# takahiroharada/OCLRadixSort

Hardware: AMD Instinct MI355X
Metric: Gkeys/s on uniform-random u32 keys; achieved % of HBM-read roofline (higher is better)
Workload: dtype u32; 1 GPU; Key-only RadixSort32, 67108864 uniform-random u32 keys (splitmix64 hi32, seed 123+step), 1xMI355X, in place; keys_per_gpu=67108864, parallelism=1 GPU, sort_algo=auto, digit_bits=8

## Files before the change

### oclradixsort_amd/csrc/hybrid_kernels.hpp

```cpp
#pragma once
#include <hip/hip_runtime.h>
#include <stdint.h>

#include "radix_kernels.hpp"
#include "onesweep_kernels.hpp"
#include "dict_kernels.hpp"
#include "dict_big_kernels.hpp"

namespace adlhip {

__device__ __forceinline__ bool grid_barrier(uint32_t* counter, uint32_t& target, uint32_t wgs, uint32_t* fault, bool data_fence = true)
{
    __shared__ uint32_t ok;
    if (!data_fence) asm volatile("s_waitcnt vmcnt(0)" ::: "memory");
    __syncthreads();
    if (threadIdx.x == 0) {
        if (data_fence) __builtin_amdgcn_fence(__ATOMIC_RELEASE, "agent");
        asm volatile("s_waitcnt vmcnt(0)" ::: "memory");
        __hip_atomic_fetch_add(counter, 1u, __ATOMIC_RELAXED, __HIP_MEMORY_SCOPE_AGENT);
        target += wgs;
        uint32_t spins = 0u, good = 1u;
        while (__hip_atomic_load(counter, __ATOMIC_RELAXED, __HIP_MEMORY_SCOPE_AGENT) < target) {
            if (++spins > (1u << 24)) { good = 0u; break; }
            __builtin_amdgcn_s_sleep(2);
// ... 977 lines not shown
        E* __restrict__ dst = out + seg_off[sg(seg)];
        auto prefetch_next = [&]() {
            if (more) {
                const S* __restrict__ src = in + (size_t)next * in_stride;
#pragma unroll
                for (int j = 0; j < K; ++j)
                    if ((uint32_t)(j * NT + tid) < m_next && m_next <= (uint32_t)CAP) e[j] = load_once(src + j * NT + tid);
            }
        };
        const bool sortable = m != 0u && m <= (uint32_t)CAP && low_bits != 0u;
        if (m > (uint32_t)CAP && tid == 0) atomicOr(fault + 1, 0x40000u);
#pragma unroll
        for (int i = 0; i < WPT; ++i) s_cnt[tid + i * NT] = 0u;
        lds_barrier();
        uint32_t rk2[(K + 1) / 2];
#pragma unroll
        for (int j = 0; j < (K + 1) / 2; ++j) rk2[j] = 0u;
        bool hard = false;
        if (sortable) {
#pragma unroll
            for (int j = 0; j < K; ++j) {
                if ((uint32_t)(j * NT + tid) < m) {
                    const uint32_t b = bin_of(e[j]);
                    const uint32_t hs = (b & 1u) << 4;
                    const uint32_t old = __hip_atomic_fetch_add(&s_cnt[b >> 1], 1u << hs, __ATOMIC_RELAXED, __HIP_MEMORY_SCOPE_WORKGROUP);
                    const uint32_t r = (old >> hs) & 0xffffu;
                    rk2[j >> 1] |= r << (16 * (j & 1));
                    hard |= r >= kBinLimit;
                }
            }
        }
        if (lane == 0) s_hard[w] = 0u;
        if (__any(hard) && lane == 0) s_hard[w] = 1u;
        lds_barrier();
        bool is_hard = false;
#pragma unroll
        for (int i = 0; i < NW; ++i) is_hard |= s_hard[i] != 0u;
        if (is_hard && tid == 0) hard_list[__hip_atomic_fetch_add(hard_cnt, 1u, __ATOMIC_RELAXED, __HIP_MEMORY_SCOPE_AGENT)] = seg;
        if (!is_hard && sortable) {
            {
                uint32_t wv[WPT];
                uint32_t sum = 0u;
#pragma unroll
                for (int i = 0; i < WPT; ++i) {
                    wv[i] = s_cnt[tid * WPT + i];
                    sum += (wv[i] & 0xffffu) + (wv[i] >> 16);
                }
                const uint32_t inc = wave_incl_scan_u32(sum);
                if (lane == 63) s_wsum[w] = inc;
                lds_barrier();
                uint32_t run = inc - sum;
#pragma unroll
                for (int i = 0; i < NW; ++i)
                    if (i < w) run += s_wsum[i];
#pragma unroll
                for (int i = 0; i < WPT; ++i) {
                    const uint32_t c0 = wv[i] & 0xffffu, c1 = wv[i] >> 16;
                    const uint32_t lo = run;
                    run += c0;
                    const uint32_t hi = run;
                    run += c1;
                    s_cnt[tid * WPT + i] = lo | (hi << 16);
                }
            }
            lds_barrier();
#pragma unroll
            for (int j = 0; j < K; ++j)
                if ((uint32_t)(j * NT + tid) < m) s_buf[(uint32_t)s_start[bin_of(e[j])] + ((rk2[j >> 1] >> (16 * (j & 1))) & 0xffffu)] = e[j];
            prefetch_next();
            lds_barrier();
#pragma unroll
            for (int j = 0; j < K; ++j) {
                const uint32_t p = (uint32_t)(j * NT + tid);
                if (p < m) {
                    const S x = s_buf[p];
                    const uint32_t b = bin_of(x);
                    const uint32_t lo = s_start[b];
                    const uint32_t hi = b == dmask ? m : (uint32_t)s_start[b + 1u];
                    uint32_t f = p;
                    if (hi - lo > 1u) {
                        uint32_t c = 0u;
                        for (uint32_t q = lo; q < hi; ++q) {
                            const S y = s_buf[q];
                            c += (y < x || (y == x && q < p)) ? 1u : 0u;
                        }
                        f = lo + c;
                    }
                    dst[f] = (E)x | hi_bits;
                }
            }
            lds_barrier();
        } else {
            if (!is_hard && m != 0u && m <= (uint32_t)CAP) {
#pragma unroll
                for (int j = 0; j < K; ++j) {
                    const uint32_t p = (uint32_t)(j * NT + tid);
                    if (p < m) dst[p] = (E)e[j] | hi_bits;
                }
            }
            prefetch_next();
        }
        if (!more) break;
        seg = next;
        m = m_next;
    }
}

struct StablePlace {
    uint32_t top;
    uint32_t low_bits;
    uint32_t sort_bits;
    uint32_t pad;
    unsigned long long prefix;
    unsigned long long kmask;
};

template <bool KEY64, typename E>
__device__ __forceinline__ unsigned long long key_of(E e)
{
    if constexpr (KEY64) return (unsigned long long)e;
    else return (unsigned long long)(uint32_t)e;
}

template <typename E>
struct BucketPass {
    const E* src;
    E* dst;
    uint32_t* cursors;
    uint32_t cursor_shift;
    uint32_t src_count_shift;
    uint32_t* flag;
    const uint32_t* src_counts;
    uint32_t n;
    uint32_t src_stride;
    uint32_t tiles_per_bucket;
    uint32_t dst_stride;
    uint32_t dst_total;
    int start_bit;
    uint32_t* zero_me;
    const uint32_t* sample;
    int which_digit;
    int dst16;
    const StablePlace* place;
    const uint32_t* status_a;
    uint32_t pieces, rows_per_chain_a, slice;
    uint32_t seg_shift;
    uint32_t* tickets;
};

struct Msd2Placement {
    int top;
    unsigned long long prefix;
};
__device__ __forceinline__ Msd2Placement msd2_placement(const uint32_t* __restrict__ sample )
{
    const unsigned long long o = ((unsigned long long)sample[1] << 32) | sample[0];
    const unsigned long long a = ((unsigned long long)sample[3] << 32) | sample[2];
    const unsigned long long diff = o ^ a;
    Msd2Placement p;
    p.top = diff ? 64 - __builtin_clzll(diff) : 0;
    if (p.top < 16) p.top = 16;
    p.prefix = p.top < 64 ? (o >> p.top) : 0ull;
    return p;
}
__device__ __forceinline__ size_t probe_sample_index(uint32_t k, uint32_t n)
{
    const uint32_t cell = n >> 14;
    const uint32_t hash24 = (uint32_t)(((unsigned long long)k * 0x9E3779B97F4A7C15ull) >> 40);
    const uint32_t jit = (uint32_t)(((unsigned long long)hash24 * cell) >> 24);
    unsigned long long at = (unsigned long long)k * (unsigned long long)n / 16384ull + jit;
    if (at >= n) at = n - 1u;
    return (size_t)at;
}
ADLHIP_KERNEL __global__ __launch_bounds__(1024) void probe_positions_selftest_kernel(uint32_t n, uint32_t* __restrict__ out)
{
    uint32_t hi = 0u, bad = 0u;
    for (int i = 0; i < 16; ++i) {
        const uint32_t k = threadIdx.x * 16u + (uint32_t)i;
        const unsigned long long at = probe_sample_index(k, n);
        const unsigned long long lo = (unsigned long long)k * n / 16384ull, up = (unsigned long long)(k + 1u) * n / 16384ull;
        if (at < lo || at >= (up > lo ? up : lo + 1ull) || at >= n) ++bad;
        hi = at > hi ? (uint32_t)at : hi;
    }
    atomicMax(out + 0, hi);
    if (bad) atomicAdd(out + 1, bad);
}

constexpr int kSampleWGs = 16;
constexpr int kSamples = 2048;
constexpr int kSampleArriveWord = 13;

__device__ __forceinline__ size_t sample_position(int k, uint32_t n)
{
    const unsigned long long lo = (unsigned long long)k * n / (unsigned)kSamples, hi = (unsigned long long)(k + 1) * n / (unsigned)kSamples;
    uint32_t h = (uint32_t)k * 0x85EBCA6Bu + 0x27D4EB2Fu;
    h ^= h >> 15;
    h *= 0xC2B2AE35u;
    h ^= h >> 13;
    return (size_t)(lo + (((unsigned long long)h * (hi - lo)) >> 32));
}

__device__ __forceinline__ void sample_accumulate(unsigned long long v0, unsigned long long v1, uint32_t* sample, uint32_t* flag)
{
    const int lane = (int)threadIdx.x;
    unsigned long long o = v0 | v1, a = v0 & v1;
#pragma unroll
    for (int sh = 32; sh >= 1; sh >>= 1) {
        o |= __shfl_xor(o, sh);
        a &= __shfl_xor(a, sh);
    }
    if (lane == 0) {
        __hip_atomic_fetch_or(sample + 0, (uint32_t)o, __ATOMIC_RELAXED, __HIP_MEMORY_SCOPE_AGENT);
        __hip_atomic_fetch_or(sample + 1, (uint32_t)(o >> 32), __ATOMIC_RELAXED, __HIP_MEMORY_SCOPE_AGENT);
        __hip_atomic_fetch_and(sample + 2, (uint32_t)a, __ATOMIC_RELAXED, __HIP_MEMORY_SCOPE_AGENT);
        __hip_atomic_fetch_and(sample + 3, (uint32_t)(a >> 32), __ATOMIC_RELAXED, __HIP_MEMORY_SCOPE_AGENT);
    }
    __shared__ uint32_t s_seen[256];
#pragma unroll
    for (int i = 0; i < 4; ++i) s_seen[i * 64 + lane] = 0u;
    uint32_t mine = 0u;
#pragma unroll
    for (int j = 0; j < 2; ++j) {
        const unsigned long long hv = ((j ? v1 : v0) + 0x632BE59BD9B4E019ull) * 0x9E3779B97F4A7C15ull;
        const uint32_t fp = (uint32_t)(hv >> 32) | 1u;
        uint32_t h = (uint32_t)(hv >> 24) & 255u;
        for (int step = 0; step < 256; ++step) {
            const uint32_t old = atomicCAS(&s_seen[h], 0u, fp);
            if (old == 0u) break;
            if (old == fp) {
                ++mine;
                break;
            }
            h = (h + 1u) & 255u;
        }
    }
    uint32_t reps = mine;
#pragma unroll
    for (int sh = 32; sh >= 1; sh >>= 1) reps += __shfl_xor(reps, sh);
    if (lane == 0 && reps) __hip_atomic_fetch_add(flag + kSampleRepeatsWord, reps, __ATOMIC_RELAXED, __HIP_MEMORY_SCOPE_AGENT);
}

template <typename E>
__global__ __launch_bounds__(64) void msd2_sample_kernel(const E* __restrict__ src, uint32_t n, uint32_t* sample, uint32_t* bar,
                                                         uint32_t* fault, uint32_t* flag, uint32_t dup_thr)
{
    const int tid = (int)(blockIdx.x * 64u + threadIdx.x);
    if (tid == 0) {
        __hip_atomic_store(bar, 0u, __ATOMIC_RELAXED, __HIP_MEMORY_SCOPE_AGENT);
        fault[0] = 0u;
        __hip_atomic_store(flag + kSampleThresholdWord, dup_thr, __ATOMIC_RELAXED, __HIP_MEMORY_SCOPE_AGENT);
    }
    if (tid < kTileTicketCounters)
        __hip_atomic_store(flag + kTileTicketWord0 + kTileTicketStride * tid, 0u, __ATOMIC_RELAXED, __HIP_MEMORY_SCOPE_AGENT);
    const E x0 = src[sample_position(2 * tid, n)], x1 = src[sample_position(2 * tid + 1, n)];
    sample_accumulate((unsigned long long)x0, (unsigned long long)x1, sample, flag);
}

template <typename E, int NT, int K, int PASS>
__global__ __launch_bounds__(NT) void msd_bucket_scatter_kernel(BucketPass<E> a)
{
    using C = TileCfg<E, 8, NT, K>;
    typedef AosIO<E> IO;
    constexpr int BINS = 256;
    constexpr int NW = C::NW;
    extern __shared__ __attribute__((aligned(16))) unsigned char smem[];
    E* __restrict__ s_elems = reinterpret_cast<E*>(smem + C::OFF_ELEMS);
    uint32_t* __restrict__ s_wcnt = reinterpret_cast<uint32_t*>(smem + C::OFF_WCNT);
    uint32_t* __restrict__ s_goff = reinterpret_cast<uint32_t*>(smem + C::OFF_GOFF);
    if (a.zero_me && blockIdx.x == 0 && threadIdx.x == 0) __hip_atomic_store(a.zero_me, 0u, __ATOMIC_RELAXED, __HIP_MEMORY_SCOPE_AGENT);
    uint32_t give_up = 0u;
    if constexpr (PASS >= 1) {
        if (threadIdx.x == 0) give_up = large_sort_gave_up(a.flag);
    }
    uint32_t base, valid, cursor_base = 0u;
    uint32_t lin = 0u;
    if constexpr (PASS == 3) {
        uint32_t* __restrict__ s_misc = reinterpret_cast<uint32_t*>(smem + C::OFF_MISC);
        const uint32_t b = blockIdx.x / a.tiles_per_bucket, t = blockIdx.x % a.tiles_per_bucket;
        if (threadIdx.x < 64u) {
            const int l = (int)threadIdx.x;
            uint32_t cnt = 0u;
            if ((uint32_t)l < a.pieces) {
                const uint32_t c0 = (uint32_t)l * a.slice;
                if (c0 < a.n) {
                    const uint32_t len = (c0 + a.slice < a.n ? c0 + a.slice : a.n) - c0;
                    const uint32_t rows = (len + (uint32_t)C::TILE - 1u) / (uint32_t)C::TILE;
                    cnt = a.status_a[((size_t)l * a.rows_per_chain_a + rows - 1u) * BINS + b] & kValMask;
                    if (cnt > a.src_stride) cnt = a.src_stride;
                }
            }
            const uint32_t incl = wave_incl_scan_u32(cnt);
            const uint32_t total = (uint32_t)__builtin_amdgcn_readlane((int)incl, 63);
            if (l < 32) {
                const bool real = (uint32_t)l < a.pieces;
                s_goff[l] = real ? incl : 0xffffffffu;
                s_goff[32 + l] = real ? (b * a.pieces + (uint32_t)l) * a.src_stride - (incl - cnt) : 0u;
            }
            const uint32_t pos = t * (uint32_t)C::TILE;
            uint32_t v = 0u;
            if (pos < total) v = total - pos < (uint32_t)C::TILE ? total - pos : (uint32_t)C::TILE;
            const unsigned long long after = __ballot((uint32_t)l < a.pieces && incl > pos && cnt != 0u);
            uint32_t ln = 0xffffffffu, split = 0u, ln2 = 0u;
            if (after && v != 0u) {
                const int c0 = __builtin_ctzll(after);
                const uint32_t end0 = (uint32_t)__builtin_amdgcn_readlane((int)incl, c0);
                const uint32_t first0 = end0 - (uint32_t)__builtin_amdgcn_readlane((int)cnt, c0);
                const unsigned long long rest = after & ~(1ull << c0);
                if (pos + v <= end0) {
                    ln = (b * a.pieces + (uint32_t)c0) * a.src_stride + (pos - first0);
                    split = v;
                } else if (rest) {
                    const int c1 = __builtin_ctzll(rest);
                    const uint32_t end1 = (uint32_t)__builtin_amdgcn_readlane((int)incl, c1);
                    if (pos + v <= end1) {
                        ln = (b * a.pieces + (uint32_t)c0) * a.src_stride + (pos - first0);
                        split = end0 - pos;
// ... 53 lines not shown
        uint32_t c = 0u;
        for (uint32_t i = 0; i < a.pieces; ++i) c += (q0 >= s_end[i]) ? 1u : 0u;
        const int rem = (int)valid - (int)wbase;
#pragma unroll
        for (int j = 0; j < K; ++j) {
            const uint32_t q = q0 + (uint32_t)(j * 64);
            while (c < 31u && q >= s_end[c]) ++c;
            e[j] = (j * 64 < rem) ? load_once(a.src + (size_t)(q + s_adj[c])) : ~E(0);
        }
    } else if (PASS == 3 && reinterpret_cast<const uint32_t*>(smem + C::OFF_MISC)[4] < valid) {
        const uint32_t split = reinterpret_cast<const uint32_t*>(smem + C::OFF_MISC)[4];
        const uint32_t ln2 = reinterpret_cast<const uint32_t*>(smem + C::OFF_MISC)[5];
        const int rem = (int)valid - (int)wbase;
#pragma unroll
        for (int j = 0; j < K; ++j) {
            const uint32_t i = wbase + (uint32_t)(j * 64);
            e[j] = (j * 64 < rem) ? load_once(a.src + (size_t)((i < split ? lin : ln2) + i)) : ~E(0);
        }
    } else {
        const typename IO::Cursor p = io.cursor((size_t)(PASS == 3 ? lin : base) + wbase);
        if (valid == (uint32_t)C::TILE) {
#pragma unroll
            for (int j = 0; j < K; ++j) e[j] = p.at(j * 64);
        } else {
            const int rem = (int)valid - (int)wbase;
#pragma unroll
            for (int j = 0; j < K; ++j) e[j] = (j * 64 < rem) ? p.at(j * 64) : ~E(0);
        }
    }
    if (a.sample && a.which_digit == 1 && place.top < (int)(8 * sizeof(E))) {
        const E pre = (E)place.prefix;
        const int rem = (int)valid - (int)wbase;
        E bad = E(0);
#pragma unroll
        for (int j = 0; j < K; ++j)
            if (j * 64 < rem) bad |= (e[j] >> place.top) ^ pre;
        if (bad != E(0)) __hip_atomic_fetch_or(a.flag, 1u, __ATOMIC_RELAXED, __HIP_MEMORY_SCOPE_AGENT);
    }
#pragma unroll
    for (int b = lane; b < BINS; b += 64) my_wcnt[b] = 0u;
    uint32_t rnk2[(K + 1) / 2];
    {
        uint32_t rnk[K];
        rank_in_wave<E, 8, K, 1>(e, rnk, my_wcnt, start_bit);
#pragma unroll
        for (int j = 0; j < K; j += 2) rnk2[j >> 1] = rnk[j] | ((j + 1 < K ? rnk[j + 1] : 0u) << 16);
    }
#pragma unroll
    for (int j = 0; j < (K + 1) / 2; ++j) asm volatile("" : "+v"(rnk2[j]));
#pragma unroll
    for (int j = 0; j < K; ++j) asm volatile("" : "+v"(e[j]));
    if constexpr (PASS >= 1) {
        if (threadIdx.x == 0) reinterpret_cast<uint32_t*>(smem + C::OFF_MISC)[8] = give_up;
    }
    __syncthreads();
    if constexpr (PASS >= 1) {
        if (reinterpret_cast<const uint32_t*>(smem + C::OFF_MISC)[8]) return;
    }
    u32x4 cnt4 = {0u, 0u, 0u, 0u};
    u32x4 toff4 = {0u, 0u, 0u, 0u};
    uint16_t* __restrict__ my_wpos = reinterpret_cast<uint16_t*>(smem + C::OFF_WPOS) + w * BINS;
    {
        u32x4 pre4 = {0u, 0u, 0u, 0u};
#pragma unroll
        for (int i = 0; i < NW; ++i) {
            const u32x4 r = *reinterpret_cast<const u32x4*>(s_wcnt + i * BINS + 4 * lane);
            cnt4 += r;
            if (i < w) pre4 += r;
        }
        const uint32_t s4 = cnt4.x + cnt4.y + cnt4.z + cnt4.w;
        const uint32_t ex = wave_incl_scan_u32(s4) - s4;
        toff4.x = ex;
        toff4.y = ex + cnt4.x;
        toff4.z = toff4.y + cnt4.y;
        toff4.w = toff4.z + cnt4.z;
        const u32x4 p4 = toff4 + pre4;
        typedef uint32_t u32x2 __attribute__((ext_vector_type(2)));
        const u32x2 packed = {p4.x | (p4.y << 16), p4.z | (p4.w << 16)};
        *reinterpret_cast<u32x2*>(my_wpos + 4 * lane) = packed;
    }
    u32x4 at4 = {0u, 0u, 0u, 0u};
    u32x4 real4 = cnt4;
    if (w == 0) {
        if (lane == 63) real4.w -= (uint32_t)C::TILE - valid;
        uint32_t* cur = a.cursors + ((size_t)(cursor_base + 4u * (uint32_t)lane) << a.cursor_shift);
        const size_t step = (size_t)1 << a.cursor_shift;
        if (real4.x) at4.x = __hip_atomic_fetch_add(cur + 0 * step, real4.x, __ATOMIC_RELAXED, __HIP_MEMORY_SCOPE_AGENT);
        if (real4.y) at4.y = __hip_atomic_fetch_add(cur + 1 * step, real4.y, __ATOMIC_RELAXED, __HIP_MEMORY_SCOPE_AGENT);
        if (real4.z) at4.z = __hip_atomic_fetch_add(cur + 2 * step, real4.z, __ATOMIC_RELAXED, __HIP_MEMORY_SCOPE_AGENT);
        if (real4.w) at4.w = __hip_atomic_fetch_add(cur + 3 * step, real4.w, __ATOMIC_RELAXED, __HIP_MEMORY_SCOPE_AGENT);
    }
    {
        constexpr int CH = K < 8 ? K : 8;
#pragma unroll
        for (int j0 = 0; j0 < K; j0 += CH) {
            uint32_t pos[CH];
#pragma unroll
            for (int j = 0; j < CH; ++j) pos[j] = my_wpos[digit_of<8>(e[(j0 + j < K) ? j0 + j : K - 1], start_bit)];
#pragma unroll
            for (int j = 0; j < CH; ++j) {
                if (j0 + j < K) {
                    const uint32_t r = (rnk2[(j0 + j) >> 1] >> (16 * ((j0 + j) & 1))) & 0xffffu;
                    s_elems[pos[j] + r] = e[j0 + j];
                }
            }
        }
    }
    if (w == 0) {
        const bool over = (at4.x + real4.x > a.dst_stride) | (at4.y + real4.y > a.dst_stride) | (at4.z + real4.z > a.dst_stride) |
                          (at4.w + real4.w > a.dst_stride);
        if (over) __hip_atomic_fetch_or(a.flag, 1u, __ATOMIC_RELAXED, __HIP_MEMORY_SCOPE_AGENT);
        uint32_t d0 = cursor_base + 4u * (uint32_t)lane;
        if constexpr (PASS >= 2)
            d0 = ((cursor_base >> 8) << a.seg_shift) + ((4u * (uint32_t)lane) & ((1u << a.seg_shift) - 1u));
        u32x4 go;
        go.x = (d0 + 0u) * a.dst_stride + at4.x - toff4.x;
        go.y = (d0 + 1u) * a.dst_stride + at4.y - toff4.y;
        go.z = (d0 + 2u) * a.dst_stride + at4.z - toff4.z;
        go.w = (d0 + 3u) * a.dst_stride + at4.w - toff4.w;
        *reinterpret_cast<u32x4*>(s_goff + 4 * lane) = (scaled && !a.dst16) ? go * (uint32_t)IO::kStoreScale : go;
    }
    __syncthreads();
    if (a.dst16) {
        uint16_t* __restrict__ d16 = reinterpret_cast<uint16_t*>(a.dst);
#pragma unroll 8
        for (int i = 0; i < K; ++i) {
            const uint32_t pos = (uint32_t)(tid + i * NT);
            if (pos < valid) {
                const E v = s_elems[pos];
                const uint32_t g = s_goff[digit_of<8>(v, start_bit)] + pos;
                if (g < a.dst_total) d16[g] = (uint16_t)v;
            }
        }
        return;
    }
    write_out_tile<IO, 8, NT, K, ADLHIP_WRITE_UNROLL>(io, s_elems, s_goff, valid, a.dst_total, start_bit, scaled);
}

template <typename E, int NT, int K>
__global__ __launch_bounds__(NT) void msd2_offsets_kernel(uint32_t* cursors_a, uint32_t* cursors_b, uint32_t* flag, uint32_t* done,
                                                          uint32_t* bar, uint32_t* __restrict__ seg_cnt, uint32_t* __restrict__ seg_off,
                                                          uint32_t* __restrict__ mode, uint32_t n,
                                                          uint32_t* sample, E* data, E* tmp, uint32_t* __restrict__ ctable,
                                                          uint32_t* fault, int key_bits, uint32_t d2_shift ,
                                                          DictBlock* dict , uint32_t* stats,
                                                          OsNet os)
{
    static_assert(NT >= 256, "one thread per digit");
    __shared__ uint32_t s_wsum[NT / 64 + 1];
    __shared__ uint32_t s_misc[4];
    extern __shared__ __attribute__((aligned(16))) unsigned char smem[];
    const int t = (int)threadIdx.x;
    const uint32_t b = blockIdx.x;
    const uint32_t overflow = large_sort_gave_up(flag);
    const uint32_t sample_repeats = __hip_atomic_load(flag + kSampleRepeatsWord, __ATOMIC_RELAXED, __HIP_MEMORY_SCOPE_AGENT);
    if (b < 256u) {
        const uint32_t ca = t < 256 ? __hip_atomic_load(cursors_a + 32 * t, __ATOMIC_RELAXED, __HIP_MEMORY_SCOPE_AGENT) : 0u;
        const uint32_t exa = block_excl_scan_u32<NT>(ca, s_wsum, nullptr);
        if (t == (int)b) s_misc[0] = exa;
        const uint32_t cb = t < 256 ? __hip_atomic_load(cursors_b + b * 256u + (uint32_t)t, __ATOMIC_RELAXED, __HIP_MEMORY_SCOPE_AGENT) : 0u;
        const uint32_t exb = block_excl_scan_u32<NT>(cb, s_wsum, nullptr);
        __syncthreads();
        if (t < 256) {
            seg_cnt[b * 256u + (uint32_t)t] = cb;
            seg_off[b * 256u + (uint32_t)t] = s_misc[0] + exb;
            __hip_atomic_store(cursors_b + b * 256u + (uint32_t)t, 0u, __ATOMIC_RELAXED, __HIP_MEMORY_SCOPE_AGENT);
        }
    }
    if (t == 0) s_misc[1] = __hip_atomic_fetch_add(done, 1u, __ATOMIC_RELAXED, __HIP_MEMORY_SCOPE_AGENT);
    __syncthreads();
    if (s_misc[1] == gridDim.x - 1u) {
        if (t < 256) __hip_atomic_store(cursors_a + 32 * t, 0u, __ATOMIC_RELAXED, __HIP_MEMORY_SCOPE_AGENT);
        if (t == 0) {
            *mode = overflow ? 1u : 0u;
            mode[kDynHardCnt] = 0u;
            seg_off[65536] = n;
            if (sample) {
                mode[kDynLowBits] = (uint32_t)(msd2_placement(sample).top - 16) + d2_shift;
                mode[kDynLowBits + 1] = (uint32_t)msd2_placement(sample).prefix;
                __hip_atomic_store(sample + 0, 0u, __ATOMIC_RELAXED, __HIP_MEMORY_SCOPE_AGENT);
                __hip_atomic_store(sample + 1, 0u, __ATOMIC_RELAXED, __HIP_MEMORY_SCOPE_AGENT);
                __hip_atomic_store(sample + 2, ~0u, __ATOMIC_RELAXED, __HIP_MEMORY_SCOPE_AGENT);
                __hip_atomic_store(sample + 3, ~0u, __ATOMIC_RELAXED, __HIP_MEMORY_SCOPE_AGENT);
            }
            __hip_atomic_store(flag, 0u, __ATOMIC_RELAXED, __HIP_MEMORY_SCOPE_AGENT);
            __hip_atomic_store(flag + kSampleRepeatsWord, 0u, __ATOMIC_RELAXED, __HIP_MEMORY_SCOPE_AGENT);
            __hip_atomic_store(done, 0u, __ATOMIC_RELAXED, __HIP_MEMORY_SCOPE_AGENT);
        }
    }
    if (overflow) {
        __syncthreads();
        net_sort<E, NT, K, 1, (int)sizeof(E)>(data, tmp, n, ctable, bar, fault, smem, key_bits, dict, stats, os, sample_repeats);
    }
}

template <typename E, bool KEY64>
__global__ __launch_bounds__(64) void msd2s_prep_kernel(const E* __restrict__ src, uint32_t n, StablePlace* __restrict__ place,
                                                         uint32_t* __restrict__ tickets, uint32_t ticket_words, uint32_t* bar,
                                                         uint32_t* fault, uint32_t sort_bits, uint32_t* flag, uint32_t dup_thr)
{
    const int tid = (int)(blockIdx.x * 64u + threadIdx.x);
    if (tid == 0) {
        __hip_atomic_store(bar, 0u, __ATOMIC_RELAXED, __HIP_MEMORY_SCOPE_AGENT);
        fault[0] = 0u;
        __hip_atomic_store(flag + kSampleThresholdWord, dup_thr, __ATOMIC_RELAXED, __HIP_MEMORY_SCOPE_AGENT);
    }
    const unsigned long long kmask = sort_bits >= 64u ? ~0ull : ((1ull << sort_bits) - 1ull);
    const E x0 = src[sample_position(2 * tid, n)], x1 = src[sample_position(2 * tid + 1, n)];
    for (uint32_t i = (uint32_t)tid; i < ticket_words; i += 64u * (uint32_t)kSampleWGs) tickets[i] = 0u;
    uint32_t* sample = flag + 8;
    sample_accumulate(key_of<KEY64>(x0) & kmask, key_of<KEY64>(x1) & kmask, sample, flag);
    asm volatile("s_waitcnt vmcnt(0)" ::: "memory");
    uint32_t arrived = 0u;
    if (threadIdx.x == 0) arrived = __hip_atomic_fetch_add(flag + kSampleArriveWord, 1u, __ATOMIC_RELAXED, __HIP_MEMORY_SCOPE_AGENT);
    if ((uint32_t)__builtin_amdgcn_readfirstlane((int)arrived) != (uint32_t)kSampleWGs - 1u) return;
    if (threadIdx.x == 0) {
        __hip_atomic_store(flag + kSampleArriveWord, 0u, __ATOMIC_RELAXED, __HIP_MEMORY_SCOPE_AGENT);
        const unsigned long long o = ((unsigned long long)__hip_atomic_load(sample + 1, __ATOMIC_RELAXED, __HIP_MEMORY_SCOPE_AGENT) << 32) |
                                     __hip_atomic_load(sample + 0, __ATOMIC_RELAXED, __HIP_MEMORY_SCOPE_AGENT);
        const unsigned long long a = ((unsigned long long)__hip_atomic_load(sample + 3, __ATOMIC_RELAXED, __HIP_MEMORY_SCOPE_AGENT) << 32) |
                                     __hip_atomic_load(sample + 2, __ATOMIC_RELAXED, __HIP_MEMORY_SCOPE_AGENT);
        __hip_atomic_store(sample + 0, 0u, __ATOMIC_RELAXED, __HIP_MEMORY_SCOPE_AGENT);
        __hip_atomic_store(sample + 1, 0u, __ATOMIC_RELAXED, __HIP_MEMORY_SCOPE_AGENT);
        __hip_atomic_store(sample + 2, ~0u, __ATOMIC_RELAXED, __HIP_MEMORY_SCOPE_AGENT);
        __hip_atomic_store(sample + 3, ~0u, __ATOMIC_RELAXED, __HIP_MEMORY_SCOPE_AGENT);
        const unsigned long long diff = o ^ a;
        uint32_t top = diff ? 64u - (uint32_t)__builtin_clzll(diff) : 0u;
        if (top < 16u) top = 16u;
        place->top = top;
        place->prefix = top < 64u ? (o >> top) : 0ull;
        place->low_bits = top - 16u;
        place->sort_bits = sort_bits;
        place->kmask = kmask;
    }
}

template <typename E>
struct LookbackPass {
    const E* src;
    E* dst;
    uint32_t* status;
    uint32_t status_bytes;
    uint32_t* tickets;
    uint32_t* flag;
    uint32_t* fault;
    const StablePlace* place;
    int which_digit;
    uint32_t n;
    uint32_t chains;
    uint32_t pieces;
    uint32_t rows_per_chain;
    uint32_t slice;
    uint32_t src_stride;
    const uint32_t* status_a;
    uint32_t rows_per_chain_a;
    uint32_t dst_stride;
    uint32_t dst_total;
    const uint32_t* soa_keys;
    const uint32_t* soa_vals;
    int dst16;
    uint32_t seg_shift;
};

template <typename E, int NT, int K, bool KEY64, int RANK = 1>
__global__ __launch_bounds__(NT) void msd_lookback_scatter_kernel(LookbackPass<E> a)
{
    using C = TileCfg<E, 8, NT, K>;
    typedef AosIO<E> IO;
    constexpr int BINS = 256;
    constexpr int NW = C::NW;
    extern __shared__ __attribute__((aligned(16))) unsigned char smem[];
    E* __restrict__ s_elems = reinterpret_cast<E*>(smem + C::OFF_ELEMS);
    uint32_t* __restrict__ s_wcnt = reinterpret_cast<uint32_t*>(smem + C::OFF_WCNT);
    uint32_t* __restrict__ s_goff = reinterpret_cast<uint32_t*>(smem + C::OFF_GOFF);
    uint32_t* __restrict__ s_misc = reinterpret_cast<uint32_t*>(smem + C::OFF_MISC);
    const int tid = (int)threadIdx.x;
    const int lane = tid & 63;
    const int w = tid >> 6;
    const uint32_t chain = a.which_digit == 2 ? blockIdx.x / a.rows_per_chain : blockIdx.x % a.chains;
    const int start_bit = (int)a.place->top - 8 * a.which_digit + (a.which_digit == 2 ? 8 - (int)a.seg_shift : 0);

    if (w == 0) {
        const bool give_up = __builtin_amdgcn_readfirstlane((int)large_sort_gave_up(a.flag)) != 0;
        uint32_t index = 0u;
        if (lane == 0 && !give_up) index = atomicAdd(&a.tickets[chain * (uint32_t)kTicketStride], 1u);
        index = (uint32_t)__builtin_amdgcn_readfirstlane((int)index);
        uint32_t base = 0u, valid = 0u;
        if (give_up) {
        } else if (a.which_digit == 1) {
            const uint32_t c0 = chain * a.slice;
            const uint32_t c1 = c0 + a.slice < a.n ? c0 + a.slice : a.n;
            const uint32_t off = index * (uint32_t)C::TILE;
            if (c0 < a.n && off < c1 - c0) {
                base = c0 + off;
                valid = c1 - base < (uint32_t)C::TILE ? c1 - base : (uint32_t)C::TILE;
            }
        } else {
            uint32_t cnt = 0u;
            if ((uint32_t)lane < a.pieces) {
                const uint32_t c0 = (uint32_t)lane * a.slice;
                if (c0 < a.n) {
                    const uint32_t len = (c0 + a.slice < a.n ? c0 + a.slice : a.n) - c0;
                    const uint32_t rows = (len + (uint32_t)C::TILE - 1u) / (uint32_t)C::TILE;
                    cnt = a.status_a[((size_t)lane * a.rows_per_chain_a + rows - 1u) * BINS + chain] & kValMask;
                    if (cnt > a.src_stride) cnt = a.src_stride;
                }
            }
            const uint32_t incl = wave_incl_scan_u32(cnt);
            const uint32_t total = (uint32_t)__builtin_amdgcn_readlane((int)incl, 63);
            if (lane < 32) {
                const bool real = (uint32_t)lane < a.pieces;
                s_goff[lane] = real ? incl : 0xffffffffu;
                s_goff[32 + lane] = real ? (chain * a.pieces + (uint32_t)lane) * a.src_stride - (incl - cnt) : 0u;
// ... 412 lines not shown
```

### oclradixsort_amd/csrc/persist_kernels.hpp

```cpp
#pragma once
#include <hip/hip_runtime.h>
#include <stdint.h>

#include "hybrid_kernels.hpp"

namespace adlhip {

template <typename E, int NT, int K>
struct PersistCfg {
    static constexpr int NW = NT / 64;
    static constexpr int TILE = NT * K;
    static constexpr int VEC = 16 / (int)sizeof(E);
    static_assert(K % VEC == 0, "whole 16-byte loads");
    static_assert(TILE <= 65536, "16-bit tile positions");
    static constexpr size_t OFF_ELEMS = 0;
    static constexpr size_t OFF_WCNT = sizeof(E) * TILE;
    static constexpr size_t OFF_WPOS = OFF_WCNT + sizeof(uint32_t) * NW * 256;
    static constexpr size_t OFF_GOFF = OFF_WPOS + sizeof(uint16_t) * NW * 256;
    static constexpr size_t OFF_PREF = OFF_GOFF + sizeof(uint32_t) * 256;
    static constexpr size_t OFF_BCNT = OFF_PREF + sizeof(uint32_t) * 260;
    static constexpr size_t OFF_WSUM = OFF_BCNT + sizeof(uint32_t) * 256;
    static constexpr size_t LDS_BYTES = OFF_WSUM + 64;
};

struct PersistTile {
    uint32_t base;
    uint32_t valid;
    uint32_t cursor_base;
};

template <typename E, int B>
__device__ __forceinline__ void rank_batch(const E* e, uint32_t* rnk, uint32_t* my_wcnt, int start_bit)
{
    const uint32_t dg0 = digit_of<8>(e[0], start_bit);
    const uint32_t d0 = (uint32_t)__builtin_amdgcn_readfirstlane((int)dg0);
    bool same = false;
    if (__all(dg0 == d0)) {
        same = true;
#pragma unroll
        for (int j = 1; j < B; ++j) same &= digit_of<8>(e[j], start_bit) == d0;
    }
    const uint32_t left = (uint32_t)__builtin_amdgcn_update_dpp((int)~dg0, (int)dg0, 0x111, 0xf, 0xf, false);
    const bool few_runs = __popcll(__ballot(left != dg0)) <= 8;
    const bool dominant = __popcll(__ballot(dg0 == d0)) >= 40;
    const int peel = few_runs ? 4 : (dominant ? 1 : 0);
    if (__all(same)) {
        uint32_t old = 0u;
        if (lane_id() == 0) old = __hip_atomic_fetch_add(&my_wcnt[d0], (uint32_t)(64 * B), __ATOMIC_RELAXED, __HIP_MEMORY_SCOPE_WORKGROUP);
        old = (uint32_t)__builtin_amdgcn_readfirstlane((int)old);
#pragma unroll
        for (int j = 0; j < B; ++j) rnk[j] = old + (uint32_t)(j * 64 + lane_id());
    } else if (peel) {
#pragma unroll
        for (int j = 0; j < B; ++j) {
            const uint32_t d = digit_of<8>(e[j], start_bit);
            uint64_t todo = __ballot(true);
            uint32_t r = 0u;
#pragma unroll 1
            for (int it = 0; it < peel && todo; ++it) {
                const uint64_t m0 = few_runs ? todo : __ballot(d == d0);
                if (!m0) break;
                const int lead = __builtin_ctzll(m0);
                const uint32_t dl = (uint32_t)__builtin_amdgcn_readlane((int)d, lead);
                const uint64_t m = __ballot(d == dl);
                uint32_t old = 0u;
                if (lane_id() == lead)
                    old = __hip_atomic_fetch_add(&my_wcnt[dl], (uint32_t)__popcll(m), __ATOMIC_RELAXED, __HIP_MEMORY_SCOPE_WORKGROUP);
                old = (uint32_t)__builtin_amdgcn_readlane((int)old, lead);
                if (d == dl) r = old + mbcnt64(m);
                todo &= ~m;
            }
            if ((todo >> lane_id()) & 1ull) r = __hip_atomic_fetch_add(&my_wcnt[d], 1u, __ATOMIC_RELAXED, __HIP_MEMORY_SCOPE_WORKGROUP);
            rnk[j] = r;
        }
    } else {
#pragma unroll
        for (int j = 0; j < B; ++j)
            rnk[j] = __hip_atomic_fetch_add(&my_wcnt[digit_of<8>(e[j], start_bit)], 1u, __ATOMIC_RELAXED, __HIP_MEMORY_SCOPE_WORKGROUP);
    }
}

template <typename E, int NT, int K, int PASS, int WPE, bool D16, int LAUX = 0, int SAUX = 0, bool DYN = false>
__global__ __launch_bounds__(NT, WPE) void msd_scatter_persist_kernel(BucketPass<E> a)
{
    using C = PersistCfg<E, NT, K>;
    constexpr int NW = C::NW;
    constexpr int TILE = C::TILE;
    constexpr int VEC = C::VEC;
    constexpr int Q = K / VEC;
    extern __shared__ __attribute__((aligned(16))) unsigned char smem[];
    E* __restrict__ s_elems = reinterpret_cast<E*>(smem + C::OFF_ELEMS);
    uint32_t* __restrict__ s_wcnt = reinterpret_cast<uint32_t*>(smem + C::OFF_WCNT);
    uint32_t* __restrict__ s_goff = reinterpret_cast<uint32_t*>(smem + C::OFF_GOFF);
    uint32_t* __restrict__ s_pref = reinterpret_cast<uint32_t*>(smem + C::OFF_PREF);
    uint32_t* __restrict__ s_bcnt = reinterpret_cast<uint32_t*>(smem + C::OFF_BCNT);
    const int tid = (int)threadIdx.x;
    const int lane = tid & 63;
    const int w = tid >> 6;
    if (a.zero_me && blockIdx.x == 0 && tid == 0) __hip_atomic_store(a.zero_me, 0u, __ATOMIC_RELAXED, __HIP_MEMORY_SCOPE_AGENT);

    uint32_t* __restrict__ s_give = reinterpret_cast<uint32_t*>(smem + C::OFF_WSUM);
    {
        if (tid == 0) s_give[8] = large_sort_gave_up(a.flag);
        __syncthreads();
        if (s_give[8]) return;
        __syncthreads();
    }
    int start_bit = a.start_bit;
    Msd2Placement place{0, 0ull};
    if (a.sample) {
        place = msd2_placement(a.sample);
        start_bit = place.top - 8 * a.which_digit;
    }
    if constexpr (PASS >= 2) start_bit += 8 - (int)a.seg_shift;

    static_assert((TILE & (TILE - 1)) == 0, "remainders by mask");
    const uint32_t G = gridDim.x, g = blockIdx.x;
    uint32_t ticket, t_end, t_step, t_origin = 0u;
    [[maybe_unused]] uint32_t n_full = 0u;
    [[maybe_unused]] uint32_t* t_counter = nullptr;
    [[maybe_unused]] const uint32_t* s_rem = nullptr;
    if constexpr (PASS == 1) {
        ticket = g;
        t_end = (a.n + (uint32_t)TILE - 1u) / (uint32_t)TILE;
        t_step = G;
        if constexpr (DYN) t_counter = a.tickets + 8 * kTileTicketStride;
    } else {
        uint32_t* s_wsum = reinterpret_cast<uint32_t*>(smem + C::OFF_WSUM);
        uint32_t tiles = 0u;
        if (tid < 256) {
            const uint32_t b = (((uint32_t)tid & 31u) << 3) | ((uint32_t)tid >> 5);
            uint32_t cnt = a.src_counts[b << a.src_count_shift];
            if (cnt > a.src_stride) cnt = a.src_stride;
            s_bcnt[tid] = cnt;
            if constexpr (DYN) tiles = cnt / (uint32_t)TILE;
            else tiles = (cnt + (uint32_t)TILE - 1u) / (uint32_t)TILE;
        }
        uint32_t total;
        const uint32_t ex = block_excl_scan_u32<NT>(tiles, s_wsum, &total);
        if (tid < 256) s_pref[tid] = ex;
        if (tid == 0) s_pref[256] = total;
        __syncthreads();
        const uint32_t x = g & 7u;
        t_origin = 32u * x;
        if constexpr (DYN) {
            uint32_t* rem_list = s_bcnt + 32u * ((x + 1u) & 7u);
            s_rem = rem_list;
            if (tid < 32) {
                const uint32_t r = s_bcnt[t_origin + (uint32_t)tid] & (uint32_t)(TILE - 1);
                uint32_t rank = 0u;
                for (uint32_t q = 0u; q < 32u; ++q) {
                    const uint32_t rq = s_bcnt[t_origin + q] & (uint32_t)(TILE - 1);
                    rank += (rq > r || (rq == r && q < (uint32_t)tid)) ? 1u : 0u;
                }
                if (r) rem_list[rank] = t_origin + (uint32_t)tid;
                const uint32_t n_rem = (uint32_t)__popcll(__ballot(r != 0u));
                if (tid == 0) s_pref[257] = n_rem;
            }
            __syncthreads();
            ticket = g >> 3;
            n_full = s_pref[t_origin + 32u] - s_pref[t_origin];
            t_end = n_full + s_pref[257];
            t_step = G >> 3;
            t_counter = a.tickets + x * kTileTicketStride;
        } else {
            ticket = s_pref[t_origin] + (g >> 3);
            t_end = s_pref[t_origin + 32u];
            t_step = G >> 3;
        }
    }
    if (ticket >= t_end) return;

    auto tile_of = [&](uint32_t t) -> PersistTile {
        PersistTile r;
        if constexpr (PASS == 1) {
            r.base = t * (uint32_t)TILE;
            const uint32_t left = a.n - r.base;
            r.valid = left < (uint32_t)TILE ? left : (uint32_t)TILE;
            r.cursor_base = 0u;
        } else if constexpr (DYN) {
            uint32_t p, off;
            if (t < n_full) {
                const uint32_t T = s_pref[t_origin] + t;
                p = t_origin;
#pragma unroll
                for (uint32_t s = 16u; s >= 1u; s >>= 1)
                    if (s_pref[p + s] <= T) p += s;
                off = (T - s_pref[p]) * (uint32_t)TILE;
                r.valid = (uint32_t)TILE;
            } else {
                p = s_rem[t - n_full];
                const uint32_t cnt = s_bcnt[p];
                off = cnt & ~(uint32_t)(TILE - 1);
                r.valid = cnt - off;
            }
            p = (uint32_t)__builtin_amdgcn_readfirstlane((int)p);
            off = (uint32_t)__builtin_amdgcn_readfirstlane((int)off);
            r.valid = (uint32_t)__builtin_amdgcn_readfirstlane((int)r.valid);
            const uint32_t b = ((p & 31u) << 3) | (p >> 5);
            r.base = b * a.src_stride + off;
            r.cursor_base = b * 256u;
        } else {
            uint32_t p = t_origin;
#pragma unroll
            for (uint32_t s = 16u; s >= 1u; s >>= 1)
                if (s_pref[p + s] <= t) p += s;
            const uint32_t b = ((p & 31u) << 3) | (p >> 5);
            const uint32_t off = (t - s_pref[p]) * (uint32_t)TILE;
            const uint32_t room = s_bcnt[p] - off;
            r.base = b * a.src_stride + off;
            r.valid = room < (uint32_t)TILE ? room : (uint32_t)TILE;
            r.cursor_base = b * 256u;
        }
        return r;
    };
    const uint32_t wbase0 = (uint32_t)(w * 64 * K + lane * VEC);
    auto load_tile = [&](const PersistTile& t, E(&e)[K]) {
        uint32_t wbase = wbase0;
        asm volatile("" : "+v"(wbase));
        const __amdgpu_buffer_rsrc_t r = __builtin_amdgcn_make_buffer_rsrc(const_cast<E*>(a.src + (size_t)t.base), 0,
                                                                           (int)(t.valid * (uint32_t)sizeof(E)), 0x00020000);
        const int off = (int)(wbase * (uint32_t)sizeof(E));
#pragma unroll
        for (int q = 0; q < Q; ++q) {
            const u32x4 v = __builtin_amdgcn_raw_buffer_load_b128(r, off, q * 64 * 16, LAUX);
            if constexpr (VEC == 4) {
                e[q * 4 + 0] = v.x; e[q * 4 + 1] = v.y; e[q * 4 + 2] = v.z; e[q * 4 + 3] = v.w;
            } else {
                e[q * 2 + 0] = (E)v.x | ((E)v.y << 32);
                e[q * 2 + 1] = (E)v.z | ((E)v.w << 32);
            }
        }
    };

    uint32_t* my_wcnt = s_wcnt + w * 256;
    uint16_t* __restrict__ my_wpos = reinterpret_cast<uint16_t*>(smem + C::OFF_WPOS) + w * 256;
    constexpr uint32_t SC = D16 ? 2u : (uint32_t)sizeof(E);
    const __amdgpu_buffer_rsrc_t dst_rsrc = __builtin_amdgcn_make_buffer_rsrc(a.dst, 0, (int)(a.dst_total * SC), 0x00020000);

    E cur[K], nxt[K];
    PersistTile tc = tile_of(ticket), tn{0u, 0u, 0u};
    load_tile(tc, cur);
    static_assert(NW >= 2, "wave 1 draws the tickets");
#pragma unroll
    for (int j = 0; j < K; ++j) asm volatile("" : "+v"(cur[j]));
    uint32_t flag_prev = 0u;
    if constexpr (DYN) {
        if (ticket + t_step < t_end) tn = tile_of(ticket + t_step);
    }
    for (;;) {
        [[maybe_unused]] uint32_t ticket_n = 0u;
        bool has_next;
        if constexpr (DYN) {
            has_next = tn.valid != 0u;
        } else {
            ticket_n = ticket + t_step;
            has_next = ticket_n < t_end;
        }
        const uint32_t flag_now = __hip_atomic_load(a.flag, __ATOMIC_RELAXED, __HIP_MEMORY_SCOPE_AGENT);
        if (has_next) {
            if constexpr (!DYN) tn = tile_of(ticket_n);
            load_tile(tn, nxt);
        }
        const uint32_t valid = tc.valid;
        const bool full = valid == (uint32_t)TILE;
        uint32_t tid_v = (uint32_t)tid;
        asm volatile("" : "+v"(tid_v));
        const uint32_t wbase = (tid_v >> 6) * (uint32_t)(64 * K) + (tid_v & 63u) * (uint32_t)VEC;
        const int rem = (int)valid - (int)wbase;
        if (PASS == 1 && a.sample && place.top < (int)(8 * sizeof(E))) {
            const E pre = (E)place.prefix;
            E bad = E(0);
#pragma unroll
            for (int q = 0; q < Q; ++q)
#pragma unroll
                for (int c = 0; c < VEC; ++c)
                    if (full || q * 64 * VEC + c < rem) bad |= (cur[q * VEC + c] >> place.top) ^ pre;
            if (bad != E(0)) __hip_atomic_fetch_or(a.flag, 1u, __ATOMIC_RELAXED, __HIP_MEMORY_SCOPE_AGENT);
        }
#pragma unroll
        for (int b = lane; b < 256; b += 64) my_wcnt[b] = 0u;
        uint32_t rnk2[(K + 1) / 2];
        if (full) {
            constexpr int B = 8;
            static_assert(K % B == 0, "whole batches");
#pragma unroll
            for (int j0 = 0; j0 < K; j0 += B) {
                uint32_t rnk[B];
                rank_batch<E, B>(cur + j0, rnk, my_wcnt, start_bit);
#pragma unroll
                for (int j = 0; j < B; j += 2) rnk2[(j0 + j) >> 1] = rnk[j] | (rnk[j + 1] << 16);
            }
        } else {
#pragma unroll
            for (int j = 0; j < K; j += 2) {
                uint32_t r0 = 0u, r1 = 0u;
                if ((j / VEC) * 64 * VEC + (j % VEC) < rem)
                    r0 = __hip_atomic_fetch_add(&my_wcnt[digit_of<8>(cur[j], start_bit)], 1u, __ATOMIC_RELAXED, __HIP_MEMORY_SCOPE_WORKGROUP);
                if (((j + 1) / VEC) * 64 * VEC + ((j + 1) % VEC) < rem)
                    r1 = __hip_atomic_fetch_add(&my_wcnt[digit_of<8>(cur[j + 1], start_bit)], 1u, __ATOMIC_RELAXED, __HIP_MEMORY_SCOPE_WORKGROUP);
                rnk2[j >> 1] = r0 | (r1 << 16);
            }
        }
#pragma unroll
        for (int j = 0; j < (K + 1) / 2; ++j) asm volatile("" : "+v"(rnk2[j]));
        if (lane == 0) s_give[w] = flag_prev;
        lds_barrier();
        {
            const u32x4 g0 = *reinterpret_cast<const u32x4*>(s_give), g1 = *reinterpret_cast<const u32x4*>(s_give + 4);
            static_assert(NW <= 8, "one word per wave");
            uint32_t any = 0u;
            if (NW > 0) any |= g0.x; if (NW > 1) any |= g0.y; if (NW > 2) any |= g0.z; if (NW > 3) any |= g0.w;
            if (NW > 4) any |= g1.x; if (NW > 5) any |= g1.y; if (NW > 6) any |= g1.z; if (NW > 7) any |= g1.w;
            if (any) break;
        }
        u32x4 cnt4 = {0u, 0u, 0u, 0u};
        u32x4 toff4 = {0u, 0u, 0u, 0u};
        {
            u32x4 pre4 = {0u, 0u, 0u, 0u};
#pragma unroll
            for (int i = 0; i < NW; ++i) {
                const u32x4 r = *reinterpret_cast<const u32x4*>(s_wcnt + i * 256 + 4 * lane);
                cnt4 += r;
                if (i < w) pre4 += r;
            }
            const uint32_t s4 = cnt4.x + cnt4.y + cnt4.z + cnt4.w;
            const uint32_t ex = wave_incl_scan_u32(s4) - s4;
            toff4.x = ex;
            toff4.y = ex + cnt4.x;
            toff4.z = toff4.y + cnt4.y;
            toff4.w = toff4.z + cnt4.z;
            const u32x4 p4 = toff4 + pre4;
            typedef uint32_t u32x2 __attribute__((ext_vector_type(2)));
            const u32x2 packed = {p4.x | (p4.y << 16), p4.z | (p4.w << 16)};
            *reinterpret_cast<u32x2*>(my_wpos + 4 * lane) = packed;
        }
        u32x4 at4 = {0u, 0u, 0u, 0u};
        if (DYN ? w <= 1 : w == 0) {
            uint32_t* cp = a.cursors + ((size_t)(tc.cursor_base + 4u * (uint32_t)lane) << a.cursor_shift);
            const size_t step = (size_t)1 << a.cursor_shift;
            u32x4 add4 = cnt4;
            if constexpr (DYN) {
                if (w == 1) {
                    cp = t_counter;
                    add4 = u32x4{lane == 0 && has_next ? 1u : 0u, 0u, 0u, 0u};
                }
            }
            if (add4.x) at4.x = __hip_atomic_fetch_add(cp + 0 * step, add4.x, __ATOMIC_RELAXED, __HIP_MEMORY_SCOPE_AGENT);
            if (add4.y) at4.y = __hip_atomic_fetch_add(cp + 1 * step, add4.y, __ATOMIC_RELAXED, __HIP_MEMORY_SCOPE_AGENT);
            if (add4.z) at4.z = __hip_atomic_fetch_add(cp + 2 * step, add4.z, __ATOMIC_RELAXED, __HIP_MEMORY_SCOPE_AGENT);
            if (add4.w) at4.w = __hip_atomic_fetch_add(cp + 3 * step, add4.w, __ATOMIC_RELAXED, __HIP_MEMORY_SCOPE_AGENT);
        }
        {
            constexpr int CH = K < 8 ? K : 8;
#pragma unroll
            for (int j0 = 0; j0 < K; j0 += CH) {
                uint32_t pos[CH];
#pragma unroll
                for (int j = 0; j < CH; ++j) pos[j] = my_wpos[digit_of<8>(cur[(j0 + j < K) ? j0 + j : K - 1], start_bit)];
#pragma unroll
                for (int j = 0; j < CH; ++j) {
                    const int jj = j0 + j;
                    if (jj < K) {
                        const uint32_t r = (rnk2[jj >> 1] >> (16 * (jj & 1))) & 0xffffu;
                        if (full || (jj / VEC) * 64 * VEC + (jj % VEC) < rem) s_elems[pos[j] + r] = cur[jj];
                    }
                }
            }
        }
        asm volatile("" : "+v"(at4.x), "+v"(at4.y), "+v"(at4.z), "+v"(at4.w));
        if (w == 0) {
            const bool over = (at4.x + cnt4.x > a.dst_stride) | (at4.y + cnt4.y > a.dst_stride) | (at4.z + cnt4.z > a.dst_stride) |
                              (at4.w + cnt4.w > a.dst_stride);
            if (over) __hip_atomic_fetch_or(a.flag, 1u, __ATOMIC_RELAXED, __HIP_MEMORY_SCOPE_AGENT);
            uint32_t d0 = tc.cursor_base + 4u * (uint32_t)lane;
            if constexpr (PASS >= 2)
                d0 = ((tc.cursor_base >> 8) << a.seg_shift) + ((4u * (uint32_t)lane) & ((1u << a.seg_shift) - 1u));
            u32x4 go;
            go.x = (d0 + 0u) * a.dst_stride + at4.x - toff4.x;
            go.y = (d0 + 1u) * a.dst_stride + at4.y - toff4.y;
            go.z = (d0 + 2u) * a.dst_stride + at4.z - toff4.z;
            go.w = (d0 + 3u) * a.dst_stride + at4.w - toff4.w;
            *reinterpret_cast<u32x4*>(s_goff + 4 * lane) = go * SC;
        }
        if constexpr (DYN) {
            if (w == 1 && lane == 0) s_give[9] = 2u * t_step + at4.x;
        }
        lds_barrier();
        [[maybe_unused]] PersistTile tnn{0u, 0u, 0u};
        if constexpr (DYN) {
            const uint32_t ticket_nn = (uint32_t)__builtin_amdgcn_readfirstlane((int)s_give[9]);
            if (has_next && ticket_nn < t_end) tnn = tile_of(ticket_nn);
        }
        {
            const uint32_t tsc = tid_v * SC;
// ... 42 lines not shown
```

Baseline: 214.8 Gkeys/s.

## Overlap persistent scatter prologue loads and rank remainders with ballots

The persistent scatter kernel now issues its first tile load before the give-up check and placement setup in pass 1. It batches the flag, sample and source-count loads so their latencies overlap, cutting the number of serialized barriers. The 32x32 remainder ranking moves from a serial loop on 32 threads to ballot/popcount across all waves. The offsets kernel also hoists its cursor loads ahead of the flag checks. The point is to shorten kernel prologue latency; the cost is tighter coupling and a hard NT==512 requirement on the DYN path.

```diff
diff --git a/oclradixsort_amd/csrc/hybrid_kernels.hpp b/oclradixsort_amd/csrc/hybrid_kernels.hpp
--- a/oclradixsort_amd/csrc/hybrid_kernels.hpp
+++ b/oclradixsort_amd/csrc/hybrid_kernels.hpp
@@ -1153,16 +1153,20 @@
     int top;
     unsigned long long prefix;
 };
-__device__ __forceinline__ Msd2Placement msd2_placement(const uint32_t* __restrict__ sample )
-{
-    const unsigned long long o = ((unsigned long long)sample[1] << 32) | sample[0];
-    const unsigned long long a = ((unsigned long long)sample[3] << 32) | sample[2];
+__device__ __forceinline__ Msd2Placement msd2_placement_of(uint32_t or_lo, uint32_t or_hi, uint32_t and_lo, uint32_t and_hi)
+{
+    const unsigned long long o = ((unsigned long long)or_hi << 32) | or_lo;
+    const unsigned long long a = ((unsigned long long)and_hi << 32) | and_lo;
     const unsigned long long diff = o ^ a;
     Msd2Placement p;
     p.top = diff ? 64 - __builtin_clzll(diff) : 0;
     if (p.top < 16) p.top = 16;
     p.prefix = p.top < 64 ? (o >> p.top) : 0ull;
     return p;
+}
+__device__ __forceinline__ Msd2Placement msd2_placement(const uint32_t* __restrict__ sample )
+{
+    return msd2_placement_of(sample[0], sample[1], sample[2], sample[3]);
 }
 __device__ __forceinline__ size_t probe_sample_index(uint32_t k, uint32_t n)
 {
@@ -1522,13 +1526,16 @@
     extern __shared__ __attribute__((aligned(16))) unsigned char smem[];
     const int t = (int)threadIdx.x;
     const uint32_t b = blockIdx.x;
+    uint32_t ca = 0u, cb = 0u;
+    if (b < 256u && t < 256) {
+        ca = __hip_atomic_load(cursors_a + 32 * t, __ATOMIC_RELAXED, __HIP_MEMORY_SCOPE_AGENT);
+        cb = __hip_atomic_load(cursors_b + b * 256u + (uint32_t)t, __ATOMIC_RELAXED, __HIP_MEMORY_SCOPE_AGENT);
+    }
     const uint32_t overflow = large_sort_gave_up(flag);
     const uint32_t sample_repeats = __hip_atomic_load(flag + kSampleRepeatsWord, __ATOMIC_RELAXED, __HIP_MEMORY_SCOPE_AGENT);
     if (b < 256u) {
-        const uint32_t ca = t < 256 ? __hip_atomic_load(cursors_a + 32 * t, __ATOMIC_RELAXED, __HIP_MEMORY_SCOPE_AGENT) : 0u;
         const uint32_t exa = block_excl_scan_u32<NT>(ca, s_wsum, nullptr);
         if (t == (int)b) s_misc[0] = exa;
-        const uint32_t cb = t < 256 ? __hip_atomic_load(cursors_b + b * 256u + (uint32_t)t, __ATOMIC_RELAXED, __HIP_MEMORY_SCOPE_AGENT) : 0u;
         const uint32_t exb = block_excl_scan_u32<NT>(cb, s_wsum, nullptr);
         __syncthreads();
         if (t < 256) {
diff --git a/oclradixsort_amd/csrc/persist_kernels.hpp b/oclradixsort_amd/csrc/persist_kernels.hpp
--- a/oclradixsort_amd/csrc/persist_kernels.hpp
+++ b/oclradixsort_amd/csrc/persist_kernels.hpp
@@ -97,22 +97,6 @@
     const int tid = (int)threadIdx.x;
     const int lane = tid & 63;
     const int w = tid >> 6;
-    if (a.zero_me && blockIdx.x == 0 && tid == 0) __hip_atomic_store(a.zero_me, 0u, __ATOMIC_RELAXED, __HIP_MEMORY_SCOPE_AGENT);
-
-    uint32_t* __restrict__ s_give = reinterpret_cast<uint32_t*>(smem + C::OFF_WSUM);
-    {
-        if (tid == 0) s_give[8] = large_sort_gave_up(a.flag);
-        __syncthreads();
-        if (s_give[8]) return;
-        __syncthreads();
-    }
-    int start_bit = a.start_bit;
-    Msd2Placement place{0, 0ull};
-    if (a.sample) {
-        place = msd2_placement(a.sample);
-        start_bit = place.top - 8 * a.which_digit;
-    }
-    if constexpr (PASS >= 2) start_bit += 8 - (int)a.seg_shift;
 
     static_assert((TILE & (TILE - 1)) == 0, "remainders by mask");
     const uint32_t G = gridDim.x, g = blockIdx.x;
@@ -120,56 +104,6 @@
     [[maybe_unused]] uint32_t n_full = 0u;
     [[maybe_unused]] uint32_t* t_counter = nullptr;
     [[maybe_unused]] const uint32_t* s_rem = nullptr;
-    if constexpr (PASS == 1) {
-        ticket = g;
-        t_end = (a.n + (uint32_t)TILE - 1u) / (uint32_t)TILE;
-        t_step = G;
-        if constexpr (DYN) t_counter = a.tickets + 8 * kTileTicketStride;
-    } else {
-        uint32_t* s_wsum = reinterpret_cast<uint32_t*>(smem + C::OFF_WSUM);
-        uint32_t tiles = 0u;
-        if (tid < 256) {
-            const uint32_t b = (((uint32_t)tid & 31u) << 3) | ((uint32_t)tid >> 5);
-            uint32_t cnt = a.src_counts[b << a.src_count_shift];
-            if (cnt > a.src_stride) cnt = a.src_stride;
-            s_bcnt[tid] = cnt;
-            if constexpr (DYN) tiles = cnt / (uint32_t)TILE;
-            else tiles = (cnt + (uint32_t)TILE - 1u) / (uint32_t)TILE;
-        }
-        uint32_t total;
-        const uint32_t ex = block_excl_scan_u32<NT>(tiles, s_wsum, &total);
-        if (tid < 256) s_pref[tid] = ex;
-        if (tid == 0) s_pref[256] = total;
-        __syncthreads();
-        const uint32_t x = g & 7u;
-        t_origin = 32u * x;
-        if constexpr (DYN) {
-            uint32_t* rem_list = s_bcnt + 32u * ((x + 1u) & 7u);
-            s_rem = rem_list;
-            if (tid < 32) {
-                const uint32_t r = s_bcnt[t_origin + (uint32_t)tid] & (uint32_t)(TILE - 1);
-                uint32_t rank = 0u;
-                for (uint32_t q = 0u; q < 32u; ++q) {
-                    const uint32_t rq = s_bcnt[t_origin + q] & (uint32_t)(TILE - 1);
-                    rank += (rq > r || (rq == r && q < (uint32_t)tid)) ? 1u : 0u;
-                }
-                if (r) rem_list[rank] = t_origin + (uint32_t)tid;
-                const uint32_t n_rem = (uint32_t)__popcll(__ballot(r != 0u));
-                if (tid == 0) s_pref[257] = n_rem;
-            }
-            __syncthreads();
-            ticket = g >> 3;
-            n_full = s_pref[t_origin + 32u] - s_pref[t_origin];
-            t_end = n_full + s_pref[257];
-            t_step = G >> 3;
-            t_counter = a.tickets + x * kTileTicketStride;
-        } else {
-            ticket = s_pref[t_origin] + (g >> 3);
-            t_end = s_pref[t_origin + 32u];
-            t_step = G >> 3;
-        }
-    }
-    if (ticket >= t_end) return;
 
     auto tile_of = [&](uint32_t t) -> PersistTile {
         PersistTile r;
@@ -239,8 +173,112 @@
     const __amdgpu_buffer_rsrc_t dst_rsrc = __builtin_amdgcn_make_buffer_rsrc(a.dst, 0, (int)(a.dst_total * SC), 0x00020000);
 
     E cur[K], nxt[K];
-    PersistTile tc = tile_of(ticket), tn{0u, 0u, 0u};
-    load_tile(tc, cur);
+    PersistTile tc{0u, 0u, 0u}, tn{0u, 0u, 0u};
+
+    if constexpr (PASS == 1) {
+        ticket = g;
+        t_end = (a.n + (uint32_t)TILE - 1u) / (uint32_t)TILE;
+        t_step = G;
+        if constexpr (DYN) t_counter = a.tickets + 8 * kTileTicketStride;
+        if (ticket < t_end) tc = tile_of(ticket);
+        load_tile(tc, cur);
+    }
+    if (a.zero_me && blockIdx.x == 0 && tid == 0) __hip_atomic_store(a.zero_me, 0u, __ATOMIC_RELAXED, __HIP_MEMORY_SCOPE_AGENT);
+
+    uint32_t* __restrict__ s_give = reinterpret_cast<uint32_t*>(smem + C::OFF_WSUM);
+    constexpr int kVerdictWord = 11, kPlaceWord = 12;
+    static_assert(kPlaceWord + 4 <= 16 && NW <= 8, "the scratch has 16 words");
+    uint32_t f_over = 0u, f_reps = 0u, f_thr = 0u;
+    u32x4 smp = {0u, 0u, 0u, 0u};
+    if (tid == 0) {
+        f_over = __hip_atomic_load(a.flag, __ATOMIC_RELAXED, __HIP_MEMORY_SCOPE_AGENT);
+        f_reps = __hip_atomic_load(a.flag + kSampleRepeatsWord, __ATOMIC_RELAXED, __HIP_MEMORY_SCOPE_AGENT);
+        f_thr = __hip_atomic_load(a.flag + kSampleThresholdWord, __ATOMIC_RELAXED, __HIP_MEMORY_SCOPE_AGENT);
+        if (a.sample) {
+            smp.x = __hip_atomic_load(a.sample + 0, __ATOMIC_RELAXED, __HIP_MEMORY_SCOPE_AGENT);
+            smp.y = __hip_atomic_load(a.sample + 1, __ATOMIC_RELAXED, __HIP_MEMORY_SCOPE_AGENT);
+            smp.z = __hip_atomic_load(a.sample + 2, __ATOMIC_RELAXED, __HIP_MEMORY_SCOPE_AGENT);
+            smp.w = __hip_atomic_load(a.sample + 3, __ATOMIC_RELAXED, __HIP_MEMORY_SCOPE_AGENT);
+        }
+    }
+    [[maybe_unused]] uint32_t src_cnt = 0u;
+    if constexpr (PASS >= 2) {
+        if (tid < 256) {
+            const uint32_t b = (((uint32_t)tid & 31u) << 3) | ((uint32_t)tid >> 5);
+            src_cnt = a.src_counts[b << a.src_count_shift];
+        }
+    }
+    if (tid == 0) {
+        s_give[kVerdictWord] = f_over | (f_reps >= f_thr ? 1u : 0u);
+        *reinterpret_cast<u32x4*>(s_give + kPlaceWord) = smp;
+    }
+    if constexpr (PASS == 1) {
+        lds_barrier();
+    } else {
+        uint32_t* s_wsum = reinterpret_cast<uint32_t*>(smem + C::OFF_WSUM);
+        uint32_t tiles = 0u;
+        if (tid < 256) {
+            uint32_t cnt = src_cnt;
+            if (cnt > a.src_stride) cnt = a.src_stride;
+            s_bcnt[tid] = cnt;
+            if constexpr (DYN) tiles = cnt / (uint32_t)TILE;
+            else tiles = (cnt + (uint32_t)TILE - 1u) / (uint32_t)TILE;
+        }
+        uint32_t total;
+        const uint32_t ex = block_excl_scan_u32<NT>(tiles, s_wsum, &total);
+        if (tid < 256) s_pref[tid] = ex;
+        if (tid == 0) s_pref[256] = total;
+    }
+    if (__builtin_amdgcn_readfirstlane((int)s_give[kVerdictWord])) return;
+    int start_bit = a.start_bit;
+    Msd2Placement place{0, 0ull};
+    if (a.sample) {
+        const u32x4 sw = *reinterpret_cast<const u32x4*>(s_give + kPlaceWord);
+        place = msd2_placement_of((uint32_t)__builtin_amdgcn_readfirstlane((int)sw.x), (uint32_t)__builtin_amdgcn_readfirstlane((int)sw.y),
+                                  (uint32_t)__builtin_amdgcn_readfirstlane((int)sw.z), (uint32_t)__builtin_amdgcn_readfirstlane((int)sw.w));
+        start_bit = place.top - 8 * a.which_digit;
+    }
+    if constexpr (PASS >= 2) start_bit += 8 - (int)a.seg_shift;
+    if constexpr (PASS >= 2) {
+        const uint32_t x = g & 7u;
+        t_origin = 32u * x;
+        if constexpr (DYN) {
+            static_assert(NT == 512, "32 x 32 compares, two per thread");
+            uint32_t* rem_list = s_bcnt + 32u * ((x + 1u) & 7u);
+            s_rem = rem_list;
+            const uint32_t q = (uint32_t)lane & 31u, h = (uint32_t)lane >> 5;
+            const uint32_t i0 = 4u * (uint32_t)w + h, i1 = i0 + 2u;
+            const uint32_t rq = s_bcnt[t_origin + q] & (uint32_t)(TILE - 1);
+            const uint32_t r0 = s_bcnt[t_origin + i0] & (uint32_t)(TILE - 1);
+            const uint32_t r1 = s_bcnt[t_origin + i1] & (uint32_t)(TILE - 1);
+            const uint64_t m0 = __ballot(rq > r0 || (rq == r0 && q < i0));
+            const uint64_t m1 = __ballot(rq > r1 || (rq == r1 && q < i1));
+            const uint32_t rank0 = (uint32_t)__popc((uint32_t)(m0 >> (32u * h)));
+            const uint32_t rank1 = (uint32_t)__popc((uint32_t)(m1 >> (32u * h)));
+            if (q == 0u) {
+                if (r0) rem_list[rank0] = t_origin + i0;
+                if (r1) rem_list[rank1] = t_origin + i1;
+            }
+            const uint32_t n_rem = (uint32_t)__popc((uint32_t)__ballot(rq != 0u));
+            if (tid == 0) s_pref[257] = n_rem;
+            __syncthreads();
+            ticket = g >> 3;
+            n_full = s_pref[t_origin + 32u] - s_pref[t_origin];
+            t_end = n_full + s_pref[257];
+            t_step = G >> 3;
+            t_counter = a.tickets + x * kTileTicketStride;
+        } else {
+            __syncthreads();
+            ticket = s_pref[t_origin] + (g >> 3);
+            t_end = s_pref[t_origin + 32u];
+            t_step = G >> 3;
+        }
+    }
+    if (ticket >= t_end) return;
+    if constexpr (PASS >= 2) {
+        tc = tile_of(ticket);
+        load_tile(tc, cur);
+    }
     static_assert(NW >= 2, "wave 1 draws the tickets");
 #pragma unroll
     for (int j = 0; j < K; ++j) asm volatile("" : "+v"(cur[j]));
```

After: 216.9 Gkeys/s, median of 6. About the same (+1.0%).
